# gattia/pyfocusr

Measured on AMD Instinct MI355X. Metric: lowest-k eigenpairs/sec + KNN-correspondence wall-clock, 250k-vertex mesh pair k=5, higher is better.
Workload: dtype f64

## Files before the change

### pyfocusr_amd/csrc/pf_internal.h

```cpp
#pragma once
#include <hip/hip_runtime.h>
#include <stdint.h>
#include <atomic>
#include <map>
#include <mutex>
#include <type_traits>
#include <unordered_map>
#include <vector>

#include "../../include/pyfocusr_hip.h"
#include "pf_scratch.h"

void pf_set_error(const char* fmt, ...);

#define PF_HIP(call)                                                                          \
    do {                                                                                      \
        hipError_t e_ = (call);                                                               \
        if (e_ != hipSuccess) {                                                               \
            pf_set_error("%s:%d %s: %s", __FILE__, __LINE__, #call, hipGetErrorString(e_));   \
            (void)hipGetLastError();  \
            return PF_E_HIP;                                                                  \
        }                                                                                     \
    } while (0)

// ... 25 lines not shown
constexpr int PF_WAVE = 64;
constexpr int PF_BLOCK = 256;
constexpr int PF_DOT_CHUNK = 4096;
constexpr int PF_MAX_ROOTS = 4096;
constexpr int PF_WIN_THREADS = 1024;
constexpr int PF_WIN_GHOSTS = 1024;
constexpr int PF_WIN_MAX = 1024;
constexpr int PF_WIN_G1 = 512;
constexpr int PF_WIN_GW = 16;
constexpr int PF_STAGE_SLOTS = 8;
constexpr size_t PF_STAGE_BYTES = 32768;
constexpr int PF_WS_TMPS = 4;

inline unsigned pf_blocks(int64_t n) { return (unsigned)((n + PF_BLOCK - 1) / PF_BLOCK); }

inline int pf_index_bits(int64_t count) {
    int b = 1;
    while (b < 62 && ((int64_t)1 << b) < count) ++b;
    return b;
}

inline int pf_check_faces(const char* fn, const int32_t* faces, int64_t n_faces, int32_t vpf, int64_t n, bool distinct) {
    for (int64_t i = 0; !distinct && i < n_faces * vpf; ++i)
        PF_CHECK(faces[i] >= 0 && faces[i] < n, PF_E_ARG, "%s: face %lld references vertex %d of %lld", fn, (long long)(i / vpf),
                 faces[i], (long long)n);
    for (int64_t t = 0; distinct && t < n_faces; ++t) {
        const int32_t* f = faces + 3 * t;
        for (int j = 0; j < 3; ++j)
            PF_CHECK(f[j] >= 0 && f[j] < n, PF_E_ARG, "%s: face %lld references vertex %d of %lld", fn, (long long)t, f[j], (long long)n);
        PF_CHECK(f[0] != f[1] && f[1] != f[2] && f[0] != f[2], PF_E_DEGENERATE, "%s: face %lld repeats a vertex", fn, (long long)t);
    }
    return PF_OK;
}

inline int pf_hip_failed(const char* fn, hipError_t e) {
    (void)hipGetLastError();
    pf_set_error("%s: %s", fn, hipGetErrorString(e));
    return PF_E_HIP;
}

struct pf_knn_tree {
    DevBuf<double> pts;
    DevBuf<int32_t> orig;
    DevBuf<double> leaf_lo;
    DevBuf<double> sup_lo;
    DevBuf<int32_t> qry_order;
    void* grid = nullptr;
    unsigned long long* counters = nullptr;
    bool count_visits = false;
};

struct pf_ctx {
    int device = 0;
    hipStream_t stream = nullptr;
    void* stage_ring = nullptr;
    hipEvent_t stage_ev[8] = {nullptr, nullptr, nullptr, nullptr, nullptr, nullptr, nullptr, nullptr};
    int stage_next = 0;
    hipStream_t copy_stream = nullptr;
    hipEvent_t ev0 = nullptr, ev1 = nullptr;
    bool timing = false;
    int timing_stride = 1;
    int64_t timing_count = 0;
    uint32_t* persist_sync = nullptr;
    int32_t* persist_abort = nullptr;
    void* persist_cal = nullptr;
    double op_ms = 0.0;
    int64_t op_launches = 0;
    double op_bytes = 0.0;
    double persist_ms = 0.0, persist_bytes = 0.0, persist_lds_bytes = 0.0;
    int64_t persist_launches = 0, persist_steps = 0;
    double knn_ms = 0.0;
    double build_ms = 0.0;
    bool build_pending = false;
    DevBuf<double> knn_ref;
    DevBuf<double> knn_qry;
    DevBuf<double> knn_ref_s;
    DevBuf<double> knn_ref_soa;
    int64_t knn_ref_ld = 0;
    DevBuf<double> knn_qry_s;
    DevBuf<unsigned> knn_ref_key;
    DevBuf<unsigned> knn_qry_key;
    DevBuf<int32_t> knn_cell_start;
    int knn_res = 0;
    void* knn_grid = nullptr;
    DevBuf<int32_t> knn_ref_orig;
    DevBuf<int32_t> knn_qry_orig;
    unsigned long long* knn_ext = nullptr;
    int64_t knn_nref = 0, knn_nqry = 0;
    int32_t knn_d = 0;
    int32_t knn_k = 1;
    DevBuf<int64_t> knn_idx;
    DevBuf<double> knn_d2;
    bool knn_ready = false, knn_done = false;
    pf_knn_tree knn_tree;
    bool knn_count_on = false;
    DevBuf<unsigned long long> knn_visited;
    int64_t knn_visited_waves = 0;
    unsigned long long* wide_count = nullptr;
    bool wide_count_on = false;
    int32_t knn_mode = 0;
    struct TimedSpan {
        hipEvent_t e0, e1;
        int64_t launches;
        double bytes;
        int64_t persist_steps;
        double lds_bytes;
    };
    std::vector<TimedSpan> spans_pending;
    std::vector<std::pair<hipEvent_t, hipEvent_t>> spans_free;
    std::vector<std::pair<int32_t, double*>> pinned_pool;
    void* pinned_scratch = nullptr;
    size_t pinned_scratch_bytes = 0;
    std::vector<hipEvent_t> event_pool;
    std::multimap<size_t, void*> free_blocks;
    std::unordered_map<void*, size_t> live_blocks;
    std::mutex alloc_mutex;
    hipStream_t stream_b = nullptr;
    hipEvent_t poison_ev = nullptr;
    hipEvent_t join_ev = nullptr, fork_ev = nullptr;
    std::vector<pf_graph*> deferred;
    std::mutex deferred_mutex;
    int64_t alloc_misses = 0;
    void* pinned_scratch_b = nullptr;
    size_t pinned_scratch_b_bytes = 0;
    void* pinned_scratch_knn = nullptr;
    size_t pinned_scratch_knn_bytes = 0;
};

inline uint64_t pf_next_uid() {
    static std::atomic<uint64_t> next{1};
    return next.fetch_add(1);
}

struct pf_graph {
    hipStream_t side_stream = nullptr;
    uint64_t uid = pf_next_uid();
    pf_ctx* ctx = nullptr;
    int64_t n = 0, n_pad = 0, n_faces = 0;
    int32_t vpf = 0;
    int32_t* rowptr = nullptr;
    int32_t* col = nullptr;
    double* w = nullptr;
    int64_t nnz_w = 0;
    double* deg = nullptr;
    double* g = nullptr;
    double* sg = nullptr;
    int32_t* label = nullptr;
    int32_t* morder = nullptr;
    int32_t* mrank = nullptr;
    int32_t* perm_m = nullptr;
    int32_t* iperm_m = nullptr;
    int32_t* perm = nullptr;
    int32_t* iperm = nullptr;
    unsigned long long* order_bbox = nullptr;
    double* smooth = nullptr;
    double* stage = nullptr;
    int64_t stage_cap = 0;
    int64_t n_slices = 0, sell_entries = 0;
    int64_t* slice_ptr = nullptr;
    int32_t* scol = nullptr;
    double* sval_rw = nullptr;
    double* sval_sym = nullptr;
    double* diag = nullptr;
    int32_t* mf_col = nullptr;
    double* mf_val = nullptr;
    int32_t win_rows = 1024;
// ... 187 lines not shown
```

### pyfocusr_amd/csrc/pf_knn.hip

```cpp
#include <hipcub/hipcub.hpp>

#include <string.h>

#include <algorithm>

#include "pf_internal.h"
#include "pf_wave.h"

namespace {

constexpr int KNN_LDS_DOUBLES = 4096;

struct KnnGrid {
    int a0, a1;
    int r0, r1;
    double lo0, lo1;
    double s0, s1;
};

__device__ __forceinline__ int cell_of(double x, double lo, double scale, int r) {
    const double t = (x - lo) * scale;
    return t > 0.0 ? (t >= (double)r ? r - 1 : (int)t) : 0;
}

__global__ __launch_bounds__(PF_BLOCK) void k_extent(const double* __restrict__ pts, int64_t n, int d, unsigned long long* ext ) {
    __shared__ unsigned long long part[PF_BLOCK / PF_WAVE][32];
    const int wave = threadIdx.x / PF_WAVE;
    for (int a = 0; a < d; ++a) {
        unsigned long long lo = ~0ull, hi = 0ull;
        for (int64_t i = (int64_t)blockIdx.x * PF_BLOCK + threadIdx.x; i < n; i += (int64_t)gridDim.x * PF_BLOCK) {
            const unsigned long long e = enc_f64(pts[i * d + a]);
            lo = e < lo ? e : lo;
            hi = e > hi ? e : hi;
        }
        for (int off = PF_WAVE / 2; off > 0; off >>= 1) {
            const unsigned long long l2 = __shfl_xor(lo, off, PF_WAVE), h2 = __shfl_xor(hi, off, PF_WAVE);
            lo = l2 < lo ? l2 : lo;
            hi = h2 > hi ? h2 : hi;
        }
        if ((threadIdx.x & (PF_WAVE - 1)) == 0) {
            part[wave][a] = lo;
            part[wave][16 + a] = hi;
        }
    }
    __syncthreads();
    if ((int)threadIdx.x < 2 * d) {
        const bool is_hi = (int)threadIdx.x >= d;
        const int a = is_hi ? (int)threadIdx.x - d + 16 : (int)threadIdx.x;
        unsigned long long v = part[0][a];
        for (int w = 1; w < PF_BLOCK / PF_WAVE; ++w) {
            const unsigned long long o = part[w][a];
            v = is_hi ? (o > v ? o : v) : (o < v ? o : v);
        }
        if (is_hi)
            atomicMax(&ext[a], v);
        else
            atomicMin(&ext[a], v);
    }
}

__global__ void k_make_grid(const unsigned long long* __restrict__ ext, int d, int res, KnnGrid* g) {
    if (threadIdx.x | blockIdx.x) return;
    int b0 = 0, b1 = 0;
    double w0 = -1.0, w1 = -1.0;
    for (int a = 0; a < d; ++a) {
        const double e = dec_f64(ext[16 + a]) - dec_f64(ext[a]);
        if (e > w0) {
            w1 = w0;
            b1 = b0;
            w0 = e;
            b0 = a;
        } else if (e > w1) {
            w1 = e;
            b1 = a;
        }
    }
    if (d == 1) {
        b1 = b0;
        w1 = 0.0;
    }
    g->a0 = b0;
    g->a1 = b1;
    g->r0 = res;
    g->r1 = d == 1 ? 1 : res;
    g->lo0 = dec_f64(ext[b0]);
    g->lo1 = dec_f64(ext[b1]);
    g->s0 = (w0 > 0.0 && isfinite(w0)) ? (double)res / w0 : 0.0;
    g->s1 = (d > 1 && w1 > 0.0 && isfinite(w1)) ? (double)res / w1 : 0.0;
}

__device__ __forceinline__ unsigned spread16(unsigned v) {
    v &= 0xffffu;
    v = (v | (v << 8)) & 0x00ff00ffu;
    v = (v | (v << 4)) & 0x0f0f0f0fu;
    v = (v | (v << 2)) & 0x33333333u;
    v = (v | (v << 1)) & 0x55555555u;
    return v;
}

__global__ __launch_bounds__(PF_BLOCK) void k_cell_keys(const double* __restrict__ pts, int64_t n, int d,
                                                        const KnnGrid* __restrict__ gp, int morton, unsigned* __restrict__ keys,
                                                        int32_t* __restrict__ vals, int32_t* __restrict__ hist) {
    const int64_t i = (int64_t)blockIdx.x * PF_BLOCK + threadIdx.x;
    if (i >= n) return;
    const KnnGrid g = *gp;
    const int cx = cell_of(pts[i * d + g.a0], g.lo0, g.s0, g.r0);
    const int cy = cell_of(pts[i * d + g.a1], g.lo1, g.s1, g.r1);
    const unsigned key = morton ? (spread16((unsigned)cx) | (spread16((unsigned)cy) << 1)) : (unsigned)(cy * g.r0 + cx);
    keys[i] = key;
    if (hist) atomicAdd(&hist[key], 1);
    else vals[i] = (int32_t)i;
}

__global__ __launch_bounds__(PF_BLOCK) void k_gather_rows(const double* __restrict__ pts, const int32_t* __restrict__ order,
                                                          int64_t n, int d, double* __restrict__ out) {
    const int64_t i = (int64_t)blockIdx.x * PF_BLOCK + threadIdx.x;
    if (i >= n) return;
    const int64_t src = order[i];
    for (int c = 0; c < d; ++c) out[i * d + c] = pts[src * d + c];
}

__global__ __launch_bounds__(PF_BLOCK) void k_cell_start(const unsigned* __restrict__ keys, int64_t n, int64_t n_cells,
                                                         int32_t* __restrict__ cell_start) {
    const int64_t c = (int64_t)blockIdx.x * PF_BLOCK + threadIdx.x;
    if (c > n_cells) return;
    int64_t lo = 0, hi = n;
    while (lo < hi) {
        const int64_t mid = (lo + hi) >> 1;
        if ((int64_t)keys[mid] < c) lo = mid + 1; else hi = mid;
    }
    cell_start[c] = (int32_t)lo;
}

template <int D>
__device__ __forceinline__ double dist2(const double (&q)[D], const double* __restrict__ r) {
    double s = 0.0;
#pragma unroll
    for (int c = 0; c < D; ++c) {
        const double df = q[c] - r[c];
        const double sq = df * df;
        s = (c == 0) ? sq : s + sq;
    }
    return s;
}

template <int D, int P>
__device__ __forceinline__ double dist2_head(const double (&q)[D], const double* __restrict__ r) {
    double s = 0.0;
#pragma unroll
    for (int c = 0; c < P; ++c) {
        const double df = q[c] - r[c];
        const double sq = df * df;
        s = (c == 0) ? sq : s + sq;
    }
    return s;
}
template <int D, int P>
__device__ __forceinline__ double dist2_tail(const double (&q)[D], const double* __restrict__ r, double s) {
#pragma unroll
    for (int c = P; c < D; ++c) {
        const double df = q[c] - r[c];
        s = s + df * df;
    }
    return s;
}

template <int K>
__device__ __forceinline__ void topk_insert(double (&best)[K], int32_t (&bidx)[K], double s, int32_t o) {
    if (!(s < best[K - 1] || (s == best[K - 1] && o < bidx[K - 1]))) return;
    best[K - 1] = s;
    bidx[K - 1] = o;
#pragma unroll
    for (int j = K - 1; j > 0; --j) {
        const bool sw = best[j] < best[j - 1] || (best[j] == best[j - 1] && bidx[j] < bidx[j - 1]);
        const double ts = best[j - 1];
        const int32_t to = bidx[j - 1];
        best[j - 1] = sw ? best[j] : ts;
        bidx[j - 1] = sw ? bidx[j] : to;
        best[j] = sw ? ts : best[j];
        bidx[j] = sw ? to : bidx[j];
    }
}

template <int D, int K, int BS, int LANE_CELLS>
__global__ __launch_bounds__(BS) void k_knn_grid(const double* __restrict__ ref_s ,
                                                       const int32_t* __restrict__ ref_orig,
                                                       const int32_t* __restrict__ cell_start, int64_t n_ref,
                                                       const double* __restrict__ qry_s, const int32_t* __restrict__ qry_orig,
                                                       int64_t n_qry, const KnnGrid* __restrict__ gp,
                                                       int64_t* __restrict__ idx_out, double* __restrict__ d2_out) {
    constexpr int KNN_TILE = (BS >= 256 ? KNN_LDS_DOUBLES : KNN_LDS_DOUBLES / 4) / (D <= 8 ? 8 : 16);
    __shared__ double tile[KNN_TILE * D];
    __shared__ int32_t tile_idx[KNN_TILE];
    __shared__ int box[BS / PF_WAVE][4];
    const KnnGrid g = *gp;
    const int64_t qi = (int64_t)blockIdx.x * BS + threadIdx.x;
    const bool mine = qi < n_qry;
    const int64_t qq = mine ? qi : n_qry - 1;
    double q[D];
#pragma unroll
    for (int c = 0; c < D; ++c) q[c] = qry_s[qq * D + c];
    const double qx = qry_s[qq * D + g.a0], qy = qry_s[qq * D + g.a1];
// ... 79 lines not shown
            if (!(lx0 >= rx0 && lx1 <= rx1 && ly0 >= ry0 && ly1 <= ry1)) {
                for (int y = ly0; y <= ly1; ++y) {
                    const int32_t b = cell_start[y * g.r0 + lx0], e = cell_start[y * g.r0 + lx1 + 1];
                    for (int32_t r = b; r < e; ++r) {
                        const double s = dist2<D>(q, ref_s + (int64_t)r * D);
                        if (s <= bestk[K - 1]) {
                            const int32_t o = ref_orig[r];
                            bool seen = false;
#pragma unroll
                            for (int j = 0; j < K; ++j) seen |= (bidx[j] == o);
                            if (!seen) topk_insert<K>(bestk, bidx, s, o);
                        }
                    }
                }
            }
            if (mine) {
                const int64_t dst = qry_orig[qi];
#pragma unroll
                for (int j = 0; j < K; ++j) {
                    idx_out[dst * K + j] = bidx[j];
                    d2_out[dst * K + j] = bestk[j];
                }
            }
            return;
        }
    }
    int bx0, bx1, by0, by1;
    block_rectangle(bx0, bx1, by0, by1);

    const int mid = (by0 + by1) / 2;
    const int half = max(mid - by0, by1 - mid);
    int since_refresh = 0;
    for (int t = 0; t <= 2 * half; ++t) {
        const int y = (t & 1) ? mid + (t + 1) / 2 : mid - t / 2;
        if (y < by0 || y > by1) continue;
        const int32_t run_b = cell_start[y * g.r0 + bx0], run_e = cell_start[y * g.r0 + bx1 + 1];
        for (int32_t t0 = run_b; t0 < run_e; t0 += KNN_TILE) {
            const int cnt = (run_e - t0) < KNN_TILE ? (run_e - t0) : KNN_TILE;
            __syncthreads();
            for (int k = threadIdx.x; k < cnt * D; k += BS) tile[k] = ref_s[(int64_t)t0 * D + k];
            for (int k = threadIdx.x; k < cnt; k += BS) tile_idx[k] = ref_orig[t0 + k];
            __syncthreads();
            for (int r = 0; r < cnt; ++r) {
                double s;
                if constexpr (D >= 6) {
                    constexpr int P = D / 2;
                    s = dist2_head<D, P>(q, tile + r * D);
                    if (!__any(s <= bestk[K - 1])) continue;
                    s = dist2_tail<D, P>(q, tile + r * D, s);
                } else {
                    s = dist2<D>(q, tile + r * D);
                }
                if (s <= bestk[K - 1]) {
                    const int32_t o = tile_idx[r];
                    bool seen = false;
#pragma unroll
                    for (int j = 0; j < K; ++j) seen |= (bidx[j] == o);
                    if (!seen) topk_insert<K>(bestk, bidx, s, o);
                }
            }
        }
        since_refresh += run_e - run_b;
        if (since_refresh >= 4 * KNN_TILE && by1 - by0 >= 8) {
            since_refresh = 0;
            int nx0, nx1, ny0, ny1;
            block_rectangle(nx0, nx1, ny0, ny1);
            bx0 = max(bx0, nx0);
            bx1 = min(bx1, nx1);
            by0 = max(by0, ny0);
            by1 = min(by1, ny1);
        }
    }
    if (mine) {
        const int64_t dst = qry_orig[qi];
#pragma unroll
        for (int j = 0; j < K; ++j) {
            idx_out[dst * K + j] = bidx[j];
            d2_out[dst * K + j] = bestk[j];
        }
    }
}

constexpr int knn_group(int d) { return d <= 4 ? 8 : (d <= 8 ? 4 : 2); }

template <int D, bool COUNT = false>
__global__ __launch_bounds__(PF_BLOCK) void k_knn_coop(const double* __restrict__ soa, int64_t ld, const int32_t* __restrict__ ref_orig,
                                                       const int32_t* __restrict__ cell_start, const double* __restrict__ qry_s,
                                                       const int32_t* __restrict__ qry_orig, int64_t n_qry,
                                                       const KnnGrid* __restrict__ gp, int64_t* __restrict__ idx_out,
                                                       double* __restrict__ d2_out, unsigned long long* __restrict__ visited = nullptr) {
    constexpr int G = knn_group(D);
    unsigned long long seen = 0;
    const unsigned long long t_begin = COUNT ? __builtin_amdgcn_s_memrealtime() : 0ull;
    unsigned long long n_chunks = 0, n_scans = 0, t_scan = 0, t_bounds = 0, n_pass = 0;
    const KnnGrid g = *gp;
    const int lane = threadIdx.x & (PF_WAVE - 1);
    const int64_t group = (int64_t)blockIdx.x * (PF_BLOCK / PF_WAVE) + __builtin_amdgcn_readfirstlane((int)(threadIdx.x / PF_WAVE));
    const int64_t q0 = group * G;
    if (q0 >= n_qry) return;
    const int nq = n_qry - q0 < G ? (int)(n_qry - q0) : G;
    double q[G][D];
    double qx[G], qy[G];
    double best[G];
    int32_t bidx[G];
    int ux0 = 0x7fffffff, ux1 = -1, uy0 = 0x7fffffff, uy1 = -1;
#pragma unroll
    for (int i = 0; i < G; ++i) {
        const int64_t qi = q0 + (i < nq ? i : nq - 1);
#pragma unroll
        for (int c = 0; c < D; ++c) q[i][c] = qry_s[qi * D + c];
        qx[i] = qry_s[qi * D + g.a0];
        qy[i] = qry_s[qi * D + g.a1];
        const int cx = cell_of(qx[i], g.lo0, g.s0, g.r0), cy = cell_of(qy[i], g.lo1, g.s1, g.r1);
        ux0 = min(ux0, cx), ux1 = max(ux1, cx);
        uy0 = min(uy0, cy), uy1 = max(uy1, cy);
        best[i] = INFINITY;
        bidx[i] = 0x7fffffff;
    }
    auto scan_rows = [&](int row_of, int x0, int x1) {
        int32_t b_l = 0, e_l = 0;
        if (row_of >= 0) {
            b_l = cell_start[row_of * g.r0 + x0];
            e_l = cell_start[row_of * g.r0 + x1 + 1];
        }
        int32_t inc = (e_l - b_l + PF_WAVE - 1) >> 6;
#pragma unroll
        for (int off = 1; off < PF_WAVE; off <<= 1) {
            const int32_t up = __shfl_up(inc, off, PF_WAVE);
            if (lane >= off) inc += up;
        }
        const int32_t total = __builtin_amdgcn_readlane(inc, PF_WAVE - 1);
        if constexpr (COUNT) n_chunks += (unsigned long long)total, n_scans += 1ull;
        for (int32_t j = 0; j < total; ++j) {
            const int row = (int)__popcll(__ballot(inc <= j));
            const int32_t first = row > 0 ? __builtin_amdgcn_readlane(inc, row - 1) : 0;
            const int32_t r = __builtin_amdgcn_readlane(b_l, row) + (j - first) * PF_WAVE + lane;
            if constexpr (COUNT) seen += (unsigned long long)__popcll(__ballot(r < __builtin_amdgcn_readlane(e_l, row)));
            if (r < __builtin_amdgcn_readlane(e_l, row)) {
                double x[D];
#pragma unroll
                for (int c = 0; c < D; ++c) x[c] = soa[(int64_t)c * ld + r];
                const int32_t o = ref_orig[r];
                if constexpr (COUNT) {
                    bool pass = false;
#pragma unroll
                    for (int i = 0; i < G; ++i) {
                        double s3 = 0.0;
#pragma unroll
                        for (int c = 0; c < D; ++c)
                            if (c != g.a0 && c != g.a1) s3 += (q[i][c] - x[c]) * (q[i][c] - x[c]);
                        pass = pass || s3 <= best[i];
                    }
                    n_pass += (unsigned long long)__popcll(__ballot(pass));
                }
#pragma unroll
                for (int i = 0; i < G; ++i) {
                    double s = 0.0;
                    constexpr int P = D >= 6 ? D / 2 : D;
#pragma unroll
                    for (int c = 0; c < P; ++c) {
                        const double df = q[i][c] - x[c];
                        const double sq = df * df;
                        s = (c == 0) ? sq : s + sq;
                    }
                    if constexpr (P < D) {
                        if (!__any(s <= best[i])) continue;
#pragma unroll
                        for (int c = P; c < D; ++c) {
                            const double df = q[i][c] - x[c];
                            s = s + df * df;
                        }
                    }
                    if (s < best[i] || (s == best[i] && o < bidx[i])) {
                        best[i] = s;
                        bidx[i] = o;
                    }
                }
            }
        }
    };
    auto bounds = [&](int& bx0, int& bx1, int& by0, int& by1) -> bool {
        bool all = true;
        bx0 = 0x7fffffff, bx1 = -1, by0 = 0x7fffffff, by1 = -1;
#pragma unroll
        for (int i = 0; i < G; ++i) {
            wave_argmin(best[i], bidx[i]);
            all = all && best[i] < INFINITY;
            const double rad = sqrt(best[i]) * (1.0 + 1e-9) + 1e-300;
            double xl = qx[i] - rad, xh = qx[i] + rad, yl = qy[i] - rad, yh = qy[i] + rad;
            xl -= fabs(xl) * 1e-15;
            xh += fabs(xh) * 1e-15;
            yl -= fabs(yl) * 1e-15;
            yh += fabs(yh) * 1e-15;
            bx0 = min(bx0, cell_of(xl, g.lo0, g.s0, g.r0)), bx1 = max(bx1, cell_of(xh, g.lo0, g.s0, g.r0));
            by0 = min(by0, cell_of(yl, g.lo1, g.s1, g.r1)), by1 = max(by1, cell_of(yh, g.lo1, g.s1, g.r1));
        }
        if (!all) bx0 = 0, by0 = 0, bx1 = g.r0 - 1, by1 = g.r1 - 1;
        return all;
    };
    int x0 = 0, x1 = -1, y0 = 0, y1 = -1;
    int rx0 = 0, rx1 = -1, ry0 = 0, ry1 = -1;
    for (int ring = 1; ring <= 4; ++ring) {
        rx0 = max(ux0 - ring, 0), rx1 = min(ux1 + ring, g.r0 - 1);
        ry0 = max(uy0 - ring, 0), ry1 = min(uy1 + ring, g.r1 - 1);
        unsigned long long ta = COUNT ? __builtin_amdgcn_s_memrealtime() : 0ull;
        for (int yb = ry0; yb <= ry1; yb += PF_WAVE) scan_rows(yb + lane <= ry1 ? yb + lane : -1, rx0, rx1);
        unsigned long long tb = COUNT ? __builtin_amdgcn_s_memrealtime() : 0ull;
        const bool all_bounded = bounds(x0, x1, y0, y1);
        if constexpr (COUNT) t_scan += tb - ta, t_bounds += __builtin_amdgcn_s_memrealtime() - tb;
        if (all_bounded) break;
    }
    if (!(x0 >= rx0 && x1 <= rx1 && y0 >= ry0 && y1 <= ry1)) {
        const int mid = min(max((uy0 + uy1) / 2, y0), y1);
        int lo = mid, hi = mid - 1;
        int w = 4;
        while (lo > y0 || hi < y1) {
            const int na = max(min(w, y1 - hi), 0), nb = max(min(w, lo - y0), 0);
            unsigned long long ta = COUNT ? __builtin_amdgcn_s_memrealtime() : 0ull;
            scan_rows(lane < na ? hi + 1 + lane : (lane < na + nb ? lo - 1 - (lane - na) : -1), x0, x1);
            unsigned long long tb = COUNT ? __builtin_amdgcn_s_memrealtime() : 0ull;
            hi += na;
            lo -= nb;
            w = min(2 * w, PF_WAVE / 2);
            int nx0, nx1, ny0, ny1;
            bounds(nx0, nx1, ny0, ny1);
            if constexpr (COUNT) t_scan += tb - ta, t_bounds += __builtin_amdgcn_s_memrealtime() - tb;
            x0 = max(x0, nx0), x1 = min(x1, nx1);
            y0 = max(y0, ny0), y1 = min(y1, ny1);
        }
    }
#pragma unroll
    for (int i = 0; i < G; ++i) {
        if (lane == i && i < nq) {
            const int64_t dst = qry_orig[q0 + i];
            idx_out[dst] = bidx[i];
            d2_out[dst] = best[i];
        }
    }
    if constexpr (COUNT) {
        if (lane == 0 && visited) {
            atomicAdd(visited, seen * (unsigned long long)nq);
            unsigned long long* rec = visited + 8 + 8 * group;
            rec[0] = __builtin_amdgcn_s_memrealtime() - t_begin;
            rec[1] = seen;
            rec[2] = n_chunks;
            rec[3] = n_scans;
            rec[4] = t_scan;
            rec[5] = t_bounds;
            rec[6] = n_pass;
        }
    }
}

constexpr int64_t PF_KNN_SMALL = 16384;
constexpr int knn_small_group(int d) { return d <= 4 ? 8 : 4; }

template <int D>
__global__ __launch_bounds__(PF_BLOCK) void k_knn_small(const double* __restrict__ ref, int64_t n_ref, const double* __restrict__ qry,
                                                        int64_t n_qry, int64_t* __restrict__ idx_out, double* __restrict__ d2_out) {
    constexpr int G = knn_small_group(D);
    const int lane = threadIdx.x & (PF_WAVE - 1);
    const int64_t group = (int64_t)blockIdx.x * (PF_BLOCK / PF_WAVE) + __builtin_amdgcn_readfirstlane((int)(threadIdx.x / PF_WAVE));
    const int64_t q0 = group * G;
    if (q0 >= n_qry) return;
    const int nq = n_qry - q0 < G ? (int)(n_qry - q0) : G;
    double q[G][D], best[G];
    int32_t bidx[G];
#pragma unroll
    for (int i = 0; i < G; ++i) {
        const int64_t qi = q0 + (i < nq ? i : nq - 1);
#pragma unroll
        for (int c = 0; c < D; ++c) q[i][c] = qry[qi * D + c];
        best[i] = INFINITY;
        bidx[i] = 0x7fffffff;
    }
    for (int64_t r = lane; r < n_ref; r += PF_WAVE) {
        double x[D];
#pragma unroll
        for (int c = 0; c < D; ++c) x[c] = ref[r * D + c];
#pragma unroll
        for (int i = 0; i < G; ++i) {
            double s = 0.0;
#pragma unroll
            for (int c = 0; c < D; ++c) {
                const double df = q[i][c] - x[c];
                const double sq = df * df;
                s = (c == 0) ? sq : s + sq;
            }
            if (s < best[i]) {
                best[i] = s;
                bidx[i] = (int32_t)r;
            }
        }
    }
#pragma unroll
    for (int i = 0; i < G; ++i) {
        wave_argmin(best[i], bidx[i]);
        if (lane == i && i < nq) {
            idx_out[q0 + i] = bidx[i];
            d2_out[q0 + i] = best[i];
        }
    }
}

template <int D>
static int launch_knn_small(pf_ctx* c) {
    const int64_t groups = (c->knn_nqry + knn_small_group(D) - 1) / knn_small_group(D);
    k_knn_small<D><<<(unsigned)((groups + PF_BLOCK / PF_WAVE - 1) / (PF_BLOCK / PF_WAVE)), PF_BLOCK, 0, c->stream>>>(
        c->knn_ref.p, c->knn_nref, c->knn_qry.p, c->knn_nqry, c->knn_idx.p, c->knn_d2.p);
    PF_HIP(hipGetLastError());
    return PF_OK;
}

__global__ __launch_bounds__(PF_BLOCK) void k_gather_rows_soa(const double* __restrict__ pts, const int32_t* __restrict__ order,
                                                              int64_t n, int d, int64_t ld, double* __restrict__ out) {
    const int64_t i = (int64_t)blockIdx.x * PF_BLOCK + threadIdx.x;
    if (i >= n) return;
    const int64_t src = order[i];
    for (int c = 0; c < d; ++c) out[(int64_t)c * ld + i] = pts[src * d + c];
}

template <int D, int K>
int launch_knn_k(pf_ctx* c) {
    constexpr int BS = D <= 6 ? PF_WAVE : PF_BLOCK;
    if constexpr (K == 1 && D <= 9) {
        const int64_t waves = (c->knn_nqry + knn_group(D) - 1) / knn_group(D);
        if (c->knn_count_on) {
            const int64_t words = 8 + 8 * waves;
            PF_HIP(c->knn_visited.grow(c->stream, words));
            c->knn_visited_waves = waves;
            PF_HIP(hipMemsetAsync(c->knn_visited.p, 0, words * sizeof(unsigned long long), c->stream));
            k_knn_coop<D, true><<<(unsigned)((waves + PF_BLOCK / PF_WAVE - 1) / (PF_BLOCK / PF_WAVE)), PF_BLOCK, 0, c->stream>>>(
                c->knn_ref_soa.p, c->knn_ref_ld, c->knn_ref_orig.p, c->knn_cell_start.p, c->knn_qry_s.p, c->knn_qry_orig.p, c->knn_nqry,
                (const KnnGrid*)c->knn_grid, c->knn_idx.p, c->knn_d2.p, c->knn_visited.p);
        } else {
            k_knn_coop<D><<<(unsigned)((waves + PF_BLOCK / PF_WAVE - 1) / (PF_BLOCK / PF_WAVE)), PF_BLOCK, 0, c->stream>>>(
                c->knn_ref_soa.p, c->knn_ref_ld, c->knn_ref_orig.p, c->knn_cell_start.p, c->knn_qry_s.p, c->knn_qry_orig.p, c->knn_nqry,
                (const KnnGrid*)c->knn_grid, c->knn_idx.p, c->knn_d2.p);
        }
    } else {
        k_knn_grid<D, K, BS, 512><<<(unsigned)((c->knn_nqry + BS - 1) / BS), BS, 0, c->stream>>>(
            c->knn_ref_s.p, c->knn_ref_orig.p, c->knn_cell_start.p, c->knn_nref, c->knn_qry_s.p, c->knn_qry_orig.p, c->knn_nqry,
            (const KnnGrid*)c->knn_grid, c->knn_idx.p, c->knn_d2.p);
    }
    PF_HIP(hipGetLastError());
    return PF_OK;
}

template <int D>
int launch_knn(pf_ctx* c) {
    if (c->knn_k == 1) return launch_knn_k<D, 1>(c);
    if constexpr (D <= 4) {
        if (c->knn_k == 2) return launch_knn_k<D, 2>(c);
        if (c->knn_k == 3) return launch_knn_k<D, 3>(c);
        if (c->knn_k == 4) return launch_knn_k<D, 4>(c);
    }
    pf_set_error("pf_knn: k = %d with d = %d is not supported (k <= 4 needs d <= 4)", c->knn_k, D);
    return PF_E_ARG;
}

__global__ __launch_bounds__(PF_BLOCK) void k_bucket_scatter(const unsigned* __restrict__ keys, int64_t n, const int32_t* __restrict__ start,
                                                             int32_t* __restrict__ cursor, unsigned* __restrict__ key_out,
                                                             int32_t* __restrict__ orig_out, const double* __restrict__ pts, int d,
                                                             double* __restrict__ rows_out) {
    const int64_t i = (int64_t)blockIdx.x * PF_BLOCK + threadIdx.x;
    if (i >= n) return;
    const unsigned k = keys[i];
    const int64_t pos = start[k] + atomicAdd(&cursor[k], 1);
    key_out[pos] = k;
    orig_out[pos] = (int32_t)i;
    for (int c = 0; c < d; ++c) rows_out[pos * d + c] = pts[i * d + c];
}

int sort_points(pf_ctx* c, const double* pts, int64_t n, int d, int morton, int key_bits, unsigned* key_out, int32_t* orig_out,
                double* rows_out) {
    Scratch s(c->stream);
    unsigned* k0 = s.get<unsigned>(n);
    int64_t n_buckets = 1;
    {
        const int res = c->knn_res;
        if (morton) {
            int bits = 0;
            while ((1 << bits) < res) ++bits;
            n_buckets = (int64_t)1 << (2 * bits);
        } else {
            n_buckets = d == 1 ? res : (int64_t)res * res;
        }
    }
    int64_t bucket_max = (int64_t)1 << 22;
    if (const char* ev = getenv("PF_KNN_BUCKET_MAX")) bucket_max = atoll(ev);
    if (n_buckets <= bucket_max) {
        int32_t* hist = s.get<int32_t>(3 * n_buckets + 2);
        s.zero(hist, sizeof(int32_t) * (size_t)(3 * n_buckets + 2));
        if (s.ok()) {
            int32_t* start = hist + n_buckets + 1;
            int32_t* cursor = start + n_buckets + 1;
            k_cell_keys<<<pf_blocks(n), PF_BLOCK, 0, s.st>>>(pts, n, d, (const KnnGrid*)c->knn_grid, morton, k0, nullptr, hist);
            s.launched();
            if (s.ok() && pf_exclusive_scan_i32(s.st, hist, start, n_buckets + 1) != PF_OK) s.note(hipErrorUnknown);
            if (s.ok()) {
                k_bucket_scatter<<<pf_blocks(n), PF_BLOCK, 0, s.st>>>(k0, n, start, cursor, key_out, orig_out, pts, d, rows_out);
                s.launched();
            }
        }
    } else {
        int32_t* v0 = s.get<int32_t>(n);
        if (s.ok()) {
            k_cell_keys<<<pf_blocks(n), PF_BLOCK, 0, s.st>>>(pts, n, d, (const KnnGrid*)c->knn_grid, morton, k0, v0, nullptr);
            s.launched();
        }
        pf_sort_pairs(s, k0, key_out, v0, orig_out, n, key_bits);
        if (s.ok()) {
            k_gather_rows<<<pf_blocks(n), PF_BLOCK, 0, s.st>>>(pts, orig_out, n, d, rows_out);
            s.launched();
        }
    }
    PF_CHECK(s.ok(), PF_E_HIP, "pf_knn: %s", hipGetErrorString(s.err));
    return PF_OK;
}

}

extern "C" {

static int knn_prepare(pf_ctx* c, int64_t n_ref, int64_t n_qry, int32_t d, int32_t k) {
    PF_CHECK(c != nullptr, PF_E_ARG, "pf_knn_upload: ctx is NULL");
    PF_CHECK(k >= 1 && k <= 4 && k <= n_ref, PF_E_ARG, "pf_knn: k = %d out of range (1..4, <= n_ref)", k);
    PF_CHECK(n_ref > 0 && n_ref < ((int64_t)1 << 31) && n_qry > 0 && n_qry < ((int64_t)1 << 31) && d >= 1 && d <= 16, PF_E_ARG,
             "pf_knn_upload: n_ref %lld, n_qry %lld, d %d out of range (1 <= d <= 16)", (long long)n_ref, (long long)n_qry, d);
    PF_HIP(hipSetDevice(c->device));
    hipStream_t st = c->stream;
    c->knn_ready = c->knn_done = false;
    PF_HIP(c->knn_ref.grow(st, n_ref * 16));
    PF_HIP(c->knn_ref_s.grow(st, n_ref * 16));
    PF_HIP(c->knn_ref_key.grow(st, n_ref));
    c->knn_ref_ld = (n_ref + PF_WAVE - 1) & ~(int64_t)(PF_WAVE - 1);
    PF_HIP(c->knn_ref_soa.grow(st, c->knn_ref_ld * d));
    static const double per_cell = [] { const char* e = getenv("PF_KNN_PER_CELL"); const double v = e ? atof(e) : 0.0; return v > 0.0 ? v : 4.0; }();
    int res = (int)sqrt((double)n_ref / per_cell);
    res = res < 4 ? 4 : (res > 2048 ? 2048 : res);
    c->knn_res = res;
    PF_HIP(c->knn_cell_start.grow(st, (int64_t)res * res + 2));
    PF_HIP(c->knn_ref_orig.grow(st, n_ref));
    PF_HIP(c->knn_qry.grow(st, n_qry * 16));
    PF_HIP(c->knn_qry_s.grow(st, n_qry * 16));
    PF_HIP(c->knn_qry_key.grow(st, n_qry));
    PF_HIP(c->knn_qry_orig.grow(st, n_qry));
    PF_HIP(c->knn_idx.grow(st, n_qry * k));
    PF_HIP(c->knn_d2.grow(st, n_qry * k));
    c->knn_k = k;
    Scratch once(st);
    if (!c->knn_ext) c->knn_ext = once.keep<unsigned long long>(32);
    if (!c->knn_grid) c->knn_grid = once.keep<KnnGrid>(1);
    PF_HIP(once.err);
    c->knn_nref = n_ref;
    c->knn_nqry = n_qry;
    c->knn_d = d;
    return PF_OK;
}

struct CoordMap {
    int32_t col[16];
    double scale[16];
};
__global__ __launch_bounds__(PF_BLOCK) void k_coords_from_final(const double* __restrict__ fin, int64_t n, int32_t fc, int32_t d,
                                                                CoordMap m, double* __restrict__ out) {
    const int64_t e = (int64_t)blockIdx.x * PF_BLOCK + threadIdx.x;
    if (e >= n * d) return;
    const int64_t i = e / d;
    const int32_t c = (int32_t)(e - i * d);
    out[e] = fin[i * fc + m.col[c]] * m.scale[c];
}

static int knn_upload_k(pf_ctx* c, const double* ref, int64_t n_ref, const double* qry, int64_t n_qry, int32_t d, int32_t k) {
    PF_CHECK(c && ref && qry, PF_E_ARG, "pf_knn_upload: NULL argument");
    PF_TRY(knn_prepare(c, n_ref, n_qry, d, k));
    hipStream_t st = c->stream;
    PF_HIP(hipMemcpyAsync(c->knn_ref.p, ref, sizeof(double) * n_ref * d, hipMemcpyHostToDevice, st));
    PF_HIP(hipMemcpyAsync(c->knn_qry.p, qry, sizeof(double) * n_qry * d, hipMemcpyHostToDevice, st));
    PF_HIP(hipStreamSynchronize(st));
    c->knn_ready = true;
    return PF_OK;
}

int pf_knn_upload(pf_ctx* c, const double* ref, int64_t n_ref, const double* qry, int64_t n_qry, int32_t d) {
    return knn_upload_k(c, ref, n_ref, qry, n_qry, d, 1);
}

static int knn_search(pf_ctx* c) {
    hipStream_t st = c->stream;
    const int d = c->knn_d;
    const char* bad_d = "pf_knn_run: no search for d = %d";
    if (c->knn_k == 1 && c->knn_mode == 0 && d <= 8 && c->knn_nref <= PF_KNN_SMALL && c->knn_nqry <= PF_KNN_SMALL)
        return pf_dispatch_d<1, 8>(d, [&](auto D) { return launch_knn_small<D()>(c); }, bad_d);
    PF_TRY(pf_knn_extent(st, c->knn_ref.p, c->knn_nref, d, c->knn_ext));
    if (c->knn_k == 1 && (c->knn_mode == 2 || (c->knn_mode == 0 && d >= PF_KNN_TREE_MIN_D))) {
        if (c->knn_nqry >= 32768) PF_TRY(pf_downloads_release(c));
        return pf_knn_tree_run(c);
    }
    const int res = c->knn_res;
    const int64_t n_cells = d == 1 ? res : (int64_t)res * res;
    int cell_bits = 1;
    while (((int64_t)1 << cell_bits) < n_cells) ++cell_bits;
    k_make_grid<<<1, 1, 0, st>>>(c->knn_ext, d, res, (KnnGrid*)c->knn_grid);
    PF_HIP(hipGetLastError());
    PF_TRY(sort_points(c, c->knn_ref.p, c->knn_nref, d, 0, cell_bits, c->knn_ref_key.p, c->knn_ref_orig.p, c->knn_ref_s.p));
    k_cell_start<<<pf_blocks(n_cells + 1), PF_BLOCK, 0, st>>>(c->knn_ref_key.p, c->knn_nref, n_cells, c->knn_cell_start.p);
    PF_HIP(hipGetLastError());
    if (c->knn_k == 1) {
        k_gather_rows_soa<<<pf_blocks(c->knn_nref), PF_BLOCK, 0, st>>>(c->knn_ref.p, c->knn_ref_orig.p, c->knn_nref, d, c->knn_ref_ld, c->knn_ref_soa.p);
        PF_HIP(hipGetLastError());
    }
    PF_TRY(sort_points(c, c->knn_qry.p, c->knn_nqry, d, 1, 32, c->knn_qry_key.p, c->knn_qry_orig.p, c->knn_qry_s.p));
    if (c->knn_nqry >= 32768) PF_TRY(pf_downloads_release(c));
    return pf_dispatch_d<1, 16>(d, [&](auto D) { return launch_knn<D()>(c); }, bad_d);
}

int pf_knn_run(pf_ctx* c) {
    PF_CHECK(c != nullptr, PF_E_ARG, "pf_knn_run: ctx is NULL");
    PF_CHECK(c->knn_ready, PF_E_STATE, "pf_knn_run: no uploaded problem");
    PF_HIP(hipSetDevice(c->device));
    PF_HIP(hipEventRecord(c->ev0, c->stream));
    PF_TRY(knn_search(c));
    PF_HIP(hipEventRecord(c->ev1, c->stream));
    PF_HIP(hipEventSynchronize(c->ev1));
    float ms = 0.f;
    PF_HIP(hipEventElapsedTime(&ms, c->ev0, c->ev1));
    c->knn_ms = ms;
    c->knn_done = true;
    return PF_OK;
}

int pf_knn_count(pf_ctx* c, int32_t enable_counting, int64_t* pairs) {
    PF_CHECK(c != nullptr, PF_E_ARG, "pf_knn_count: ctx is NULL");
    unsigned long long h = 0ull;
    if (c->knn_visited.p) {
        PF_HIP(hipMemcpyAsync(&h, c->knn_visited.p, sizeof(h), hipMemcpyDeviceToHost, c->stream));
        PF_HIP(hipStreamSynchronize(c->stream));
    }
    if (pairs) *pairs = (int64_t)h;
    c->knn_count_on = enable_counting != 0;
    return PF_OK;
}

int pf_knn_wave_stats(pf_ctx* c, double* sum_us, double* max_us, int64_t* waves, int64_t* max_candidates, double* detail ) {
    PF_CHECK(c != nullptr, PF_E_ARG, "pf_knn_wave_stats: ctx is NULL");
    const int64_t nw = c->knn_visited.p ? c->knn_visited_waves : 0;
    std::vector<unsigned long long> h((size_t)(8 * nw), 0ull);
    if (nw > 0) {
        PF_HIP(hipMemcpyAsync(h.data(), c->knn_visited.p + 8, sizeof(unsigned long long) * h.size(), hipMemcpyDeviceToHost, c->stream));
        PF_HIP(hipStreamSynchronize(c->stream));
    }
    unsigned long long sum = 0, mx = 0, mc = 0, ch = 0, sc = 0, ts = 0, tb = 0, np = 0;
    for (int64_t w = 0; w < nw; ++w) {
        const unsigned long long* r = h.data() + 8 * w;
        sum += r[0];
        if (r[0] > mx) mx = r[0], mc = r[1];
        ch += r[2], sc += r[3], ts += r[4], tb += r[5], np += r[6];
    }
    if (sum_us) *sum_us = 0.01 * (double)sum;
    if (max_us) *max_us = 0.01 * (double)mx;
    if (waves) *waves = nw;
    if (max_candidates) *max_candidates = (int64_t)mc;
    if (detail) detail[0] = (double)ch, detail[1] = (double)sc, detail[2] = 0.01 * (double)ts, detail[3] = 0.01 * (double)tb, detail[4] = (double)np;
    return PF_OK;
}

int pf_knn_mode(pf_ctx* c, int32_t mode) {
    PF_CHECK(c != nullptr && mode >= 0 && mode <= 2, PF_E_ARG, "pf_knn_mode: bad argument");
    c->knn_mode = mode;
    return PF_OK;
}

int pf_knn_download(pf_ctx* c, int64_t* idx_out, double* d2_out) {
    PF_CHECK(c != nullptr && idx_out != nullptr, PF_E_ARG, "pf_knn_download: NULL argument");
    PF_CHECK(c->knn_done, PF_E_STATE, "pf_knn_download: pf_knn_run has not completed");
    PF_HIP(hipSetDevice(c->device));
    const size_t count = (size_t)c->knn_nqry * c->knn_k;
    const size_t bytes = sizeof(int64_t) * count;
    if (bytes * (d2_out ? 2 : 1) <= ((size_t)8 << 20)) {
        unsigned char* pin = nullptr;
        PF_TRY(pf_pinned_scratch(c, bytes * (d2_out ? 2 : 1), reinterpret_cast<void**>(&pin), 2));
        PF_TRY(pf_copy_by_kernel(c->stream, c->knn_idx.p, pin, bytes));
        if (d2_out) PF_TRY(pf_copy_by_kernel(c->stream, c->knn_d2.p, pin + bytes, bytes));
        PF_HIP(hipStreamSynchronize(c->stream));
        memcpy(idx_out, pin, bytes);
        if (d2_out) memcpy(d2_out, pin + bytes, bytes);
// ... 88 lines not shown
```

Baseline: 1033.

## Add third-axis slab binning to KNN grid and split spread query groups

Extends the 2D uniform grid used for exact k=1 nearest-neighbour search with a third axis of up to 32 slabs, chosen when the third-widest extent is large enough, so each cell holds fewer candidates in 3D meshes. The cooperative wave search now scans 3D boxes of cell rows with a slab-aware expansion, and rewrites row chunking into a packed prefix-sum walk over candidates instead of per-row 64-lane chunks. Query groups whose cells are far apart are searched one query at a time to avoid inflated bounding boxes. This adds more cell-start entries, a larger sort key range and more complex indexing logic in exchange for fewer distance evaluations.

```diff
diff --git a/pyfocusr_amd/csrc/pf_internal.h b/pyfocusr_amd/csrc/pf_internal.h
--- a/pyfocusr_amd/csrc/pf_internal.h
+++ b/pyfocusr_amd/csrc/pf_internal.h
@@ -131,6 +131,8 @@
     DevBuf<unsigned> knn_qry_key;
     DevBuf<int32_t> knn_cell_start;
     int knn_res = 0;
+    int knn_res3 = 0;
+    int knn_slabs = 1;
     void* knn_grid = nullptr;
     DevBuf<int32_t> knn_ref_orig;
     DevBuf<int32_t> knn_qry_orig;
diff --git a/pyfocusr_amd/csrc/pf_knn.hip b/pyfocusr_amd/csrc/pf_knn.hip
--- a/pyfocusr_amd/csrc/pf_knn.hip
+++ b/pyfocusr_amd/csrc/pf_knn.hip
@@ -12,11 +12,15 @@
 constexpr int KNN_LDS_DOUBLES = 4096;
 
 struct KnnGrid {
-    int a0, a1;
-    int r0, r1;
-    double lo0, lo1;
-    double s0, s1;
+    int a0, a1, a2;
+    int r0, r1, r2;
+    double lo0, lo1, lo2;
+    double s0, s1, s2;
 };
+
+constexpr int PF_KNN_SLABS = 32;
+constexpr double KNN_SLABS_PER_COLUMN = 2.5;
+constexpr int64_t KNN_BUCKET_MAX = (int64_t)1 << 22;
 
 __device__ __forceinline__ int cell_of(double x, double lo, double scale, int r) {
     const double t = (x - lo) * scale;
@@ -59,22 +63,39 @@
     }
 }
 
-__global__ void k_make_grid(const unsigned long long* __restrict__ ext, int d, int res, KnnGrid* g) {
+__global__ void k_make_grid(const unsigned long long* __restrict__ ext, int d, int res, int res3, int r2_max, KnnGrid* g) {
     if (threadIdx.x | blockIdx.x) return;
-    int b0 = 0, b1 = 0;
-    double w0 = -1.0, w1 = -1.0;
+    int b0 = 0, b1 = 0, b2 = 0;
+    double w0 = -1.0, w1 = -1.0, w2 = -1.0;
     for (int a = 0; a < d; ++a) {
         const double e = dec_f64(ext[16 + a]) - dec_f64(ext[a]);
         if (e > w0) {
+            w2 = w1;
+            b2 = b1;
             w1 = w0;
             b1 = b0;
             w0 = e;
             b0 = a;
         } else if (e > w1) {
+            w2 = w1;
+            b2 = b1;
             w1 = e;
             b1 = a;
-        }
-    }
+        } else if (e > w2) {
+            w2 = e;
+            b2 = a;
+        }
+    }
+    int r2 = 1;
+    if (d >= 3 && r2_max > 1 && w2 > 0.0 && isfinite(w2) && isfinite(w0)) {
+        const double fit = w2 * (double)res3 / w0;
+        if (fit >= 2.0) r2 = fit < (double)r2_max ? (int)ceil(fit) : r2_max;
+    }
+    if (r2 > 1) res = res3;
+    g->a2 = r2 > 1 ? b2 : b0;
+    g->r2 = r2;
+    g->lo2 = r2 > 1 ? dec_f64(ext[b2]) : 0.0;
+    g->s2 = r2 > 1 ? (double)r2 / w2 : 0.0;
     if (d == 1) {
         b1 = b0;
         w1 = 0.0;
@@ -106,7 +127,15 @@
     const KnnGrid g = *gp;
     const int cx = cell_of(pts[i * d + g.a0], g.lo0, g.s0, g.r0);
     const int cy = cell_of(pts[i * d + g.a1], g.lo1, g.s1, g.r1);
-    const unsigned key = morton ? (spread16((unsigned)cx) | (spread16((unsigned)cy) << 1)) : (unsigned)(cy * g.r0 + cx);
+    const int cz = g.r2 > 1 ? cell_of(pts[i * d + g.a2], g.lo2, g.s2, g.r2) : 0;
+    unsigned key;
+    if (morton) {
+        int bits = 0;
+        while ((1 << bits) < g.r0) ++bits;
+        key = spread16((unsigned)cx) | (spread16((unsigned)cy) << 1) | ((unsigned)cz << (2 * bits));
+    } else {
+        key = (unsigned)((cz * g.r1 + cy) * g.r0 + cx);
+    }
     keys[i] = key;
     if (hist) atomicAdd(&hist[key], 1);
     else vals[i] = (int32_t)i;
@@ -118,6 +147,11 @@
     if (i >= n) return;
     const int64_t src = order[i];
     for (int c = 0; c < d; ++c) out[i * d + c] = pts[src * d + c];
+}
+
+static int64_t knn_cells(const pf_ctx* c, int d) {
+    const int64_t two = (int64_t)c->knn_res * c->knn_res, three = (int64_t)c->knn_res3 * c->knn_res3 * c->knn_slabs;
+    return d == 1 ? c->knn_res : (two > three ? two : three);
 }
 
 __global__ __launch_bounds__(PF_BLOCK) void k_cell_start(const unsigned* __restrict__ keys, int64_t n, int64_t n_cells,
@@ -363,6 +397,7 @@
 }
 
 constexpr int knn_group(int d) { return d <= 4 ? 8 : (d <= 8 ? 4 : 2); }
+constexpr int KNN_GROUP_SPAN = 8;
 
 template <int D, bool COUNT = false>
 __global__ __launch_bounds__(PF_BLOCK) void k_knn_coop(const double* __restrict__ soa, int64_t ld, const int32_t* __restrict__ ref_orig,
@@ -381,43 +416,62 @@
     if (q0 >= n_qry) return;
     const int nq = n_qry - q0 < G ? (int)(n_qry - q0) : G;
     double q[G][D];
-    double qx[G], qy[G];
+    double qx[G], qy[G], qz[G];
     double best[G];
     int32_t bidx[G];
-    int ux0 = 0x7fffffff, ux1 = -1, uy0 = 0x7fffffff, uy1 = -1;
-#pragma unroll
-    for (int i = 0; i < G; ++i) {
-        const int64_t qi = q0 + (i < nq ? i : nq - 1);
-#pragma unroll
-        for (int c = 0; c < D; ++c) q[i][c] = qry_s[qi * D + c];
-        qx[i] = qry_s[qi * D + g.a0];
-        qy[i] = qry_s[qi * D + g.a1];
-        const int cx = cell_of(qx[i], g.lo0, g.s0, g.r0), cy = cell_of(qy[i], g.lo1, g.s1, g.r1);
-        ux0 = min(ux0, cx), ux1 = max(ux1, cx);
-        uy0 = min(uy0, cy), uy1 = max(uy1, cy);
-        best[i] = INFINITY;
-        bidx[i] = 0x7fffffff;
-    }
+    int ux0 = 0x7fffffff, ux1 = -1, uy0 = 0x7fffffff, uy1 = -1, uz0 = 0x7fffffff, uz1 = -1;
+    double zmin = 0.0, zmax = 0.0;
+    auto take_queries = [&](int first, int count) {
+        ux0 = 0x7fffffff, ux1 = -1, uy0 = 0x7fffffff, uy1 = -1, uz0 = 0x7fffffff, uz1 = -1;
+#pragma unroll
+        for (int i = 0; i < G; ++i) {
+            const int64_t qi = q0 + first + (i < count ? i : count - 1);
+#pragma unroll
+            for (int c = 0; c < D; ++c) q[i][c] = qry_s[qi * D + c];
+            qx[i] = qry_s[qi * D + g.a0];
+            qy[i] = qry_s[qi * D + g.a1];
+            qz[i] = qry_s[qi * D + g.a2];
+            const int cx = cell_of(qx[i], g.lo0, g.s0, g.r0), cy = cell_of(qy[i], g.lo1, g.s1, g.r1);
+            const int cz = cell_of(qz[i], g.lo2, g.s2, g.r2);
+            ux0 = min(ux0, cx), ux1 = max(ux1, cx);
+            uy0 = min(uy0, cy), uy1 = max(uy1, cy);
+            uz0 = min(uz0, cz), uz1 = max(uz1, cz);
+            zmin = i == 0 ? qz[i] : fmin(zmin, qz[i]), zmax = i == 0 ? qz[i] : fmax(zmax, qz[i]);
+            best[i] = INFINITY;
+            bidx[i] = 0x7fffffff;
+        }
+    };
     auto scan_rows = [&](int row_of, int x0, int x1) {
         int32_t b_l = 0, e_l = 0;
         if (row_of >= 0) {
             b_l = cell_start[row_of * g.r0 + x0];
             e_l = cell_start[row_of * g.r0 + x1 + 1];
         }
-        int32_t inc = (e_l - b_l + PF_WAVE - 1) >> 6;
+        int32_t inc = e_l - b_l;
+        unsigned long long rows_left = __ballot(inc > 0);
 #pragma unroll
         for (int off = 1; off < PF_WAVE; off <<= 1) {
             const int32_t up = __shfl_up(inc, off, PF_WAVE);
             if (lane >= off) inc += up;
         }
         const int32_t total = __builtin_amdgcn_readlane(inc, PF_WAVE - 1);
-        if constexpr (COUNT) n_chunks += (unsigned long long)total, n_scans += 1ull;
-        for (int32_t j = 0; j < total; ++j) {
-            const int row = (int)__popcll(__ballot(inc <= j));
-            const int32_t first = row > 0 ? __builtin_amdgcn_readlane(inc, row - 1) : 0;
-            const int32_t r = __builtin_amdgcn_readlane(b_l, row) + (j - first) * PF_WAVE + lane;
-            if constexpr (COUNT) seen += (unsigned long long)__popcll(__ballot(r < __builtin_amdgcn_readlane(e_l, row)));
-            if (r < __builtin_amdgcn_readlane(e_l, row)) {
+        const int32_t exc = inc - (e_l - b_l), off_l = b_l - exc;
+        if constexpr (COUNT) n_chunks += (unsigned long long)((total + PF_WAVE - 1) >> 6), n_scans += 1ull;
+        int32_t carry = 0;
+        for (int32_t base = 0; base < total; base += PF_WAVE) {
+            const int32_t cand = base + lane;
+            int32_t off = carry;
+            while (rows_left) {
+                const int row = (int)__builtin_ctzll(rows_left);
+                const int32_t begins = __builtin_amdgcn_readlane(exc, row);
+                if (begins >= base + PF_WAVE) break;
+                carry = __builtin_amdgcn_readlane(off_l, row);
+                off = cand >= begins ? carry : off;
+                rows_left &= rows_left - 1;
+            }
+            const int32_t r = cand + off;
+            if constexpr (COUNT) seen += (unsigned long long)__popcll(__ballot(cand < total));
+            if (cand < total) {
                 double x[D];
 #pragma unroll
                 for (int c = 0; c < D; ++c) x[c] = soa[(int64_t)c * ld + r];
@@ -429,7 +483,7 @@
                         double s3 = 0.0;
 #pragma unroll
                         for (int c = 0; c < D; ++c)
-                            if (c != g.a0 && c != g.a1) s3 += (q[i][c] - x[c]) * (q[i][c] - x[c]);
+                            if (c != g.a0 && c != g.a1 && (g.r2 == 1 || c != g.a2)) s3 += (q[i][c] - x[c]) * (q[i][c] - x[c]);
                         pass = pass || s3 <= best[i];
                     }
                     n_pass += (unsigned long long)__popcll(__ballot(pass));
@@ -460,67 +514,101 @@
             }
         }
     };
-    auto bounds = [&](int& bx0, int& bx1, int& by0, int& by1) -> bool {
+    auto bounds = [&](int& bx0, int& bx1, int& by0, int& by1, int& bz0, int& bz1) -> bool {
         bool all = true;
-        bx0 = 0x7fffffff, bx1 = -1, by0 = 0x7fffffff, by1 = -1;
+        bx0 = 0x7fffffff, bx1 = -1, by0 = 0x7fffffff, by1 = -1, bz0 = 0x7fffffff, bz1 = -1;
 #pragma unroll
         for (int i = 0; i < G; ++i) {
             wave_argmin(best[i], bidx[i]);
             all = all && best[i] < INFINITY;
             const double rad = sqrt(best[i]) * (1.0 + 1e-9) + 1e-300;
-            double xl = qx[i] - rad, xh = qx[i] + rad, yl = qy[i] - rad, yh = qy[i] + rad;
+            double xl = qx[i] - rad, xh = qx[i] + rad, yl = qy[i] - rad, yh = qy[i] + rad, zl = qz[i] - rad, zh = qz[i] + rad;
             xl -= fabs(xl) * 1e-15;
             xh += fabs(xh) * 1e-15;
             yl -= fabs(yl) * 1e-15;
             yh += fabs(yh) * 1e-15;
+            zl -= fabs(zl) * 1e-15;
+            zh += fabs(zh) * 1e-15;
             bx0 = min(bx0, cell_of(xl, g.lo0, g.s0, g.r0)), bx1 = max(bx1, cell_of(xh, g.lo0, g.s0, g.r0));
             by0 = min(by0, cell_of(yl, g.lo1, g.s1, g.r1)), by1 = max(by1, cell_of(yh, g.lo1, g.s1, g.r1));
-        }
-        if (!all) bx0 = 0, by0 = 0, bx1 = g.r0 - 1, by1 = g.r1 - 1;
+            bz0 = min(bz0, cell_of(zl, g.lo2, g.s2, g.r2)), bz1 = max(bz1, cell_of(zh, g.lo2, g.s2, g.r2));
+        }
+        if (!all) bx0 = 0, by0 = 0, bz0 = 0, bx1 = g.r0 - 1, by1 = g.r1 - 1, bz1 = g.r2 - 1;
         return all;
     };
-    int x0 = 0, x1 = -1, y0 = 0, y1 = -1;
-    int rx0 = 0, rx1 = -1, ry0 = 0, ry1 = -1;
-    for (int ring = 1; ring <= 4; ++ring) {
-        rx0 = max(ux0 - ring, 0), rx1 = min(ux1 + ring, g.r0 - 1);
-        ry0 = max(uy0 - ring, 0), ry1 = min(uy1 + ring, g.r1 - 1);
-        unsigned long long ta = COUNT ? __builtin_amdgcn_s_memrealtime() : 0ull;
-        for (int yb = ry0; yb <= ry1; yb += PF_WAVE) scan_rows(yb + lane <= ry1 ? yb + lane : -1, rx0, rx1);
-        unsigned long long tb = COUNT ? __builtin_amdgcn_s_memrealtime() : 0ull;
-        const bool all_bounded = bounds(x0, x1, y0, y1);
-        if constexpr (COUNT) t_scan += tb - ta, t_bounds += __builtin_amdgcn_s_memrealtime() - tb;
-        if (all_bounded) break;
-    }
-    if (!(x0 >= rx0 && x1 <= rx1 && y0 >= ry0 && y1 <= ry1)) {
-        const int mid = min(max((uy0 + uy1) / 2, y0), y1);
-        int lo = mid, hi = mid - 1;
-        int w = 4;
-        while (lo > y0 || hi < y1) {
-            const int na = max(min(w, y1 - hi), 0), nb = max(min(w, lo - y0), 0);
+    auto scan_box = [&](int xa, int xb, int ya, int yb, int za, int zb, int sy0, int sy1, int sz0, int sz1) {
+        const int ny = yb - ya + 1, rows = ny * (zb - za + 1);
+        for (int t0 = 0; t0 < rows; t0 += PF_WAVE) {
+            const int t = t0 + lane;
+            const int z = za + t / ny, y = ya + t % ny;
+            const bool skip = y >= sy0 && y <= sy1 && z >= sz0 && z <= sz1;
+            scan_rows(t < rows && !skip ? z * g.r1 + y : -1, xa, xb);
+        }
+    };
+    const double side = fmax(g.s0 > 0.0 ? 1.0 / g.s0 : 0.0, g.s1 > 0.0 ? 1.0 / g.s1 : 0.0);
+    take_queries(0, nq);
+    const bool apart = ux1 - ux0 > KNN_GROUP_SPAN || uy1 - uy0 > KNN_GROUP_SPAN || zmax - zmin > KNN_GROUP_SPAN * side;
+    const int count = apart ? 1 : nq;
+    unsigned long long pairs = 0;
+    for (int first = 0; first < nq; first += count) {
+        if (apart) take_queries(first, 1);
+        const unsigned long long seen_before = seen;
+        int x0 = 0, x1 = -1, y0 = 0, y1 = -1, z0 = 0, z1 = -1;
+        int rx0 = 0, rx1 = -1, ry0 = 0, ry1 = -1, rz0 = 0, rz1 = -1;
+        for (int ring = 1; ring <= 5; ++ring) {
+            int sz0 = 0, sz1 = -1;
+            if (ring <= 4) {
+                rx0 = max(ux0 - ring, 0), rx1 = min(ux1 + ring, g.r0 - 1);
+                ry0 = max(uy0 - ring, 0), ry1 = min(uy1 + ring, g.r1 - 1);
+                rz0 = cell_of(zmin - ring * side, g.lo2, g.s2, g.r2), rz1 = cell_of(zmax + ring * side, g.lo2, g.s2, g.r2);
+            } else {
+                if (rz0 == 0 && rz1 == g.r2 - 1) break;
+                sz0 = rz0, sz1 = rz1;
+                rz0 = 0, rz1 = g.r2 - 1;
+            }
             unsigned long long ta = COUNT ? __builtin_amdgcn_s_memrealtime() : 0ull;
-            scan_rows(lane < na ? hi + 1 + lane : (lane < na + nb ? lo - 1 - (lane - na) : -1), x0, x1);
+            scan_box(rx0, rx1, ry0, ry1, rz0, rz1, ry0, ry1, sz0, sz1);
             unsigned long long tb = COUNT ? __builtin_amdgcn_s_memrealtime() : 0ull;
-            hi += na;
-            lo -= nb;
-            w = min(2 * w, PF_WAVE / 2);
-            int nx0, nx1, ny0, ny1;
-            bounds(nx0, nx1, ny0, ny1);
+            const bool all_bounded = bounds(x0, x1, y0, y1, z0, z1);
             if constexpr (COUNT) t_scan += tb - ta, t_bounds += __builtin_amdgcn_s_memrealtime() - tb;
-            x0 = max(x0, nx0), x1 = min(x1, nx1);
-            y0 = max(y0, ny0), y1 = min(y1, ny1);
-        }
-    }
-#pragma unroll
-    for (int i = 0; i < G; ++i) {
-        if (lane == i && i < nq) {
-            const int64_t dst = qry_orig[q0 + i];
-            idx_out[dst] = bidx[i];
-            d2_out[dst] = best[i];
-        }
+            if (all_bounded) break;
+        }
+        if (!(x0 >= rx0 && x1 <= rx1 && y0 >= ry0 && y1 <= ry1 && z0 >= rz0 && z1 <= rz1)) {
+            const int midy = min(max((uy0 + uy1) / 2, y0), y1);
+            int ylo = midy, yhi = midy - 1, zlo = 0x7fffffff, zhi = -1;
+            int w = 4, reach = 0;
+            while (ylo > y0 || yhi < y1 || zlo > z0 || zhi < z1) {
+                reach += w;
+                const int ya = max(ylo - w, y0), yb = min(yhi + w, y1);
+                const bool rows_done = ya <= y0 && yb >= y1;
+                const int za = rows_done ? z0 : max(min(zlo, cell_of(zmin - reach * side, g.lo2, g.s2, g.r2)), z0);
+                const int zb = rows_done ? z1 : min(max(zhi, cell_of(zmax + reach * side, g.lo2, g.s2, g.r2)), z1);
+                unsigned long long ta = COUNT ? __builtin_amdgcn_s_memrealtime() : 0ull;
+                scan_box(x0, x1, ya, yb, za, zb, ylo, yhi, zlo, zhi);
+                unsigned long long tb = COUNT ? __builtin_amdgcn_s_memrealtime() : 0ull;
+                ylo = min(ylo, ya), yhi = max(yhi, yb), zlo = min(zlo, za), zhi = max(zhi, zb);
+                w = min(2 * w, PF_WAVE / 2);
+                int nx0, nx1, ny0, ny1, nz0, nz1;
+                bounds(nx0, nx1, ny0, ny1, nz0, nz1);
+                if constexpr (COUNT) t_scan += tb - ta, t_bounds += __builtin_amdgcn_s_memrealtime() - tb;
+                x0 = max(x0, nx0), x1 = min(x1, nx1);
+                y0 = max(y0, ny0), y1 = min(y1, ny1);
+                z0 = max(z0, nz0), z1 = min(z1, nz1);
+            }
+        }
+#pragma unroll
+        for (int i = 0; i < G; ++i) {
+            if (lane == i && i < count) {
+                const int64_t dst = qry_orig[q0 + first + i];
+                idx_out[dst] = bidx[i];
+                d2_out[dst] = best[i];
+            }
+        }
+        if constexpr (COUNT) pairs += (seen - seen_before) * (unsigned long long)count;
     }
     if constexpr (COUNT) {
         if (lane == 0 && visited) {
-            atomicAdd(visited, seen * (unsigned long long)nq);
+            atomicAdd(visited, pairs);
             unsigned long long* rec = visited + 8 + 8 * group;
             rec[0] = __builtin_amdgcn_s_memrealtime() - t_begin;
             rec[1] = seen;
@@ -661,14 +749,15 @@
     {
         const int res = c->knn_res;
         if (morton) {
-            int bits = 0;
+            int bits = 0, zbits = 0;
             while ((1 << bits) < res) ++bits;
-            n_buckets = (int64_t)1 << (2 * bits);
+            while ((1 << zbits) < c->knn_slabs) ++zbits;
+            n_buckets = (int64_t)1 << (2 * bits + zbits);
         } else {
-            n_buckets = d == 1 ? res : (int64_t)res * res;
-        }
-    }
-    int64_t bucket_max = (int64_t)1 << 22;
+            n_buckets = knn_cells(c, d);
+        }
+    }
+    int64_t bucket_max = KNN_BUCKET_MAX;
     if (const char* ev = getenv("PF_KNN_BUCKET_MAX")) bucket_max = atoll(ev);
     if (n_buckets <= bucket_max) {
         int32_t* hist = s.get<int32_t>(3 * n_buckets + 2);
@@ -717,11 +806,26 @@
     PF_HIP(c->knn_ref_key.grow(st, n_ref));
     c->knn_ref_ld = (n_ref + PF_WAVE - 1) & ~(int64_t)(PF_WAVE - 1);
     PF_HIP(c->knn_ref_soa.grow(st, c->knn_ref_ld * d));
-    static const double per_cell = [] { const char* e = getenv("PF_KNN_PER_CELL"); const double v = e ? atof(e) : 0.0; return v > 0.0 ? v : 4.0; }();
+    const char* pc = getenv("PF_KNN_PER_CELL");
+    const double per_cell = pc && atof(pc) > 0.0 ? atof(pc) : 4.0;
     int res = (int)sqrt((double)n_ref / per_cell);
     res = res < 4 ? 4 : (res > 2048 ? 2048 : res);
     c->knn_res = res;
-    PF_HIP(c->knn_cell_start.grow(st, (int64_t)res * res + 2));
+    int slabs = 1;
+    c->knn_res3 = res;
+    if (k == 1 && d >= 3 && d <= 9) {
+        const int res3 = (int)sqrt((double)n_ref / (per_cell * KNN_SLABS_PER_COLUMN));
+        c->knn_res3 = res3 < 4 ? 4 : res3;
+        const char* e = getenv("PF_KNN_SLABS");
+        slabs = e ? atoi(e) : PF_KNN_SLABS;
+        int bits = 0;
+        while ((1 << bits) < res) ++bits;
+        const int64_t fit = KNN_BUCKET_MAX >> (2 * bits);
+        slabs = slabs > fit ? (int)fit : slabs;
+        slabs = slabs < 1 ? 1 : slabs;
+    }
+    c->knn_slabs = slabs;
+    PF_HIP(c->knn_cell_start.grow(st, knn_cells(c, d) + 2));
     PF_HIP(c->knn_ref_orig.grow(st, n_ref));
     PF_HIP(c->knn_qry.grow(st, n_qry * 16));
     PF_HIP(c->knn_qry_s.grow(st, n_qry * 16));
@@ -780,10 +884,10 @@
         return pf_knn_tree_run(c);
     }
     const int res = c->knn_res;
-    const int64_t n_cells = d == 1 ? res : (int64_t)res * res;
+    const int64_t n_cells = knn_cells(c, d);
     int cell_bits = 1;
     while (((int64_t)1 << cell_bits) < n_cells) ++cell_bits;
-    k_make_grid<<<1, 1, 0, st>>>(c->knn_ext, d, res, (KnnGrid*)c->knn_grid);
+    k_make_grid<<<1, 1, 0, st>>>(c->knn_ext, d, res, c->knn_res3, c->knn_slabs, (KnnGrid*)c->knn_grid);
     PF_HIP(hipGetLastError());
     PF_TRY(sort_points(c, c->knn_ref.p, c->knn_nref, d, 0, cell_bits, c->knn_ref_key.p, c->knn_ref_orig.p, c->knn_ref_s.p));
     k_cell_start<<<pf_blocks(n_cells + 1), PF_BLOCK, 0, st>>>(c->knn_ref_key.p, c->knn_nref, n_cells, c->knn_cell_start.p);
```

Result: no change. 1030 (-0.3%).
